# antoyang/FrozenBiLM

Hardware: AMD Instinct MI355X
Metric: video-text samples/sec (MLM fwd+bwd) DeBERTa-XL+adapters (higher is better)
Workload: dtype bf16; 1 GPU; DeBERTa-v2-XLarge(24L)+adapters ds8/8, B=32/GPU, T=10x1024, L=256 (S=266), MLM fwd+bwd+allreduce+clip+Adam, dropout 0.1 live, seeded random weights; global_batch=32, seq_len=266, parallelism=dp1, dead_layer23_encoder_pass=skipped (output unused, SURVEY fact 6); FLOPs still counted

## Files before the change

frozenbilm_amd/csrc/attn_bwd.hip:

```cpp
#include "attn_common.h"
#include "../../include/fbl.h"

namespace {
using namespace attn;

__global__ void rowdot_kernel(const bf16* dO, const bf16* O, long ld, float* out, int B, int S, int nh) {
  const long gid = (long)blockIdx.x * blockDim.x + threadIdx.x;
  const long idx = gid >> 3;
  const int c = (int)(gid & 7);
  const long total = (long)B * S * nh;
  const bool live = idx < total;
  const long row = live ? idx / nh : 0;
  const int h = live ? (int)(idx % nh) : 0;
  float s = 0.f;
  if (live) {
    const bf16x8 x = *(const bf16x8*)(dO + row * ld + h * 64 + c * 8);
    const bf16x8 y = *(const bf16x8*)(O + row * ld + h * 64 + c * 8);
#pragma unroll
    for (int e = 0; e < 8; ++e) s += bf2f(x[e]) * bf2f(y[e]);
  }
  s += __shfl_xor(s, 1, 64);
  s += __shfl_xor(s, 2, 64);
  s += __shfl_xor(s, 4, 64);
  if (live && c == 0) {
// ... 645 lines not shown
  }
}

struct BwdQArgs {
  const bf16* dS;
  const bf16* k; long ldk;
  const bf16* pkx;
  const int32_t* klen; const int32_t* border;
  bf16* dQ; long lddq;
  int B, S, Sp, nh;
  const int32_t* row0;
};
constexpr int LDG1 = 104;
constexpr int Q_DS = 0;
constexpr int Q_KS = Q_DS + 8192;
constexpr int Q_G1 = Q_KS + 8192;
constexpr int Q_TAB = Q_G1 + 64 * LDG1 * 2;
constexpr int Q_TOTAL = Q_TAB + 16384;
static_assert(3 * Q_TOTAL <= 160 * 1024, "three workgroups per CU");

template <bool PACKED = false>
__global__ __launch_bounds__(256, 3) void attn_bwd_dq_kernel(BwdQArgs a) {
  extern __shared__ __attribute__((aligned(16))) char smem[];
  const int tid = threadIdx.x, lane = tid & 63;
  const int w = __builtin_amdgcn_readfirstlane(tid >> 6);
  const int c = lane & 15, g = lane >> 4;
  const int S = a.S, Sp = a.Sp;
  const WgCoord wc = wg_coord(Sp / 64, a.nh, a.B, a.border);
  const int i0 = wc.x * 64, h = wc.h, b = wc.b;
  const int i = i0 + w * 16 + c;
  const long rb = PACKED ? (long)a.row0[b] : (long)b * S;
  const int lim = PACKED ? min(a.row0[b + 1] - a.row0[b], S) : S;
  const int kl = a.klen ? min(a.klen[b], S) : S;
  const int nkt = (i0 < kl) ? (kl + 63) / 64 : 0;
  const int srow = tid >> 3, sch = tid & 7;
  const int sb = srow * 128 + ((sch ^ tswz(srow)) << 4);
  const int ks0 = (w < 2) ? 0 : 1;
  bf16* g1 = (bf16*)(smem + Q_G1) + (w * 16 + c) * LDG1;
  const int wr = w * 16 + c;
  f32x4 dq[4];
#pragma unroll
  for (int dt = 0; dt < 4; ++dt) dq[dt] = (f32x4){0.f, 0.f, 0.f, 0.f};
  if (nkt > 0) {
    for (int t = tid; t < (64 * LDG1 * 2) / 16; t += 256) *(bf16x8*)(smem + Q_G1 + t * 16) = (bf16x8){0, 0, 0, 0, 0, 0, 0, 0};
    __syncthreads();
  }

  const long sbase = ((long)b * a.nh + h) * Sp * Sp;
  const __amdgpu_buffer_rsrc_t sr = buf_rsrc(a.dS + sbase + (long)i0 * Sp);
  const __amdgpu_buffer_rsrc_t kr = buf_rsrc(a.k + rb * a.ldk + h * 64);
  const __amdgpu_buffer_rsrc_t xr = buf_rsrc(a.pkx + (long)h * 2 * Sp * 64);
  const uint32_t so = (uint32_t)((wr * Sp + g * 16) * 2);
  const uint32_t ldk2 = (uint32_t)(a.ldk * 2);
  const int beta0 = (i0 - 64 + Sp) >> 6;

  struct Regs { bf16x8 s[2], k[2], x[2]; } R;
  auto load_pair = [&](int jt) {
#pragma unroll
    for (int t = 0; t < 2; ++t) {
      R.s[t] = buf_ld16(sr, so + (uint32_t)(t * 16), (uint32_t)(jt * 128));
      const uint32_t jr = (uint32_t)min(jt * 64 + srow + t * 32, lim - 1);
      R.k[t] = buf_ld16(kr, jr * ldk2 + (uint32_t)(sch * 16), 0);
      R.x[t] = buf_ld16(xr, (uint32_t)((srow + t * 32) * 128 + sch * 16), (uint32_t)((beta0 - jt) * 8192));
    }
  };
  if (nkt > 0) {
    load_pair(0);
#pragma unroll
    for (int t = 0; t < 2; ++t)
      *(bf16x8*)(smem + Q_TAB + ((beta0 + 1) & 1) * 8192 + sb + t * 4096) =
          buf_ld16(xr, (uint32_t)((srow + t * 32) * 128 + sch * 16), (uint32_t)((beta0 + 1) * 8192));
  }
  for (int jt = 0; jt < nkt; ++jt) {
#pragma unroll
    for (int t = 0; t < 2; ++t) {
      *(bf16x8*)(smem + Q_KS + sb + t * 4096) = R.k[t];
      *(bf16x8*)(smem + Q_TAB + ((beta0 - jt) & 1) * 8192 + sb + t * 4096) = R.x[t];
      *(bf16x8*)(smem + Q_DS + wr * 128 + (((2 * g + t) ^ (wr & 7)) << 4)) = R.s[t];
    }
    {
      bf16* gs = g1 + wr + 64 - g * 16 - ks0 * 32;
#pragma unroll
      for (int t = 0; t < 2; ++t)
#pragma unroll
        for (int e = 0; e < 8; ++e) gs[-(t * 8 + e)] = R.s[t][e];
    }
    __syncthreads();
    load_pair(min(jt + 1, nkt - 1));
#pragma unroll
    for (int kk = 0; kk < 2; ++kk) {
      const int rk = kk * 32 + g * 8 + (c >> 2);
      const bf16x8 sf = *(const bf16x8*)(smem + Q_DS + wr * 128 + (((kk * 4 + g) ^ (wr & 7)) << 4));
#pragma unroll
      for (int dt = 0; dt < 4; ++dt) {
        const int ch = dt * 2 + ((c >> 1) & 1), sub = (c & 1) * 8;
        union { tr16x4 h[2]; bf16x8 v; } u;
        u.h[0] = lds_tr16((const bf16*)(smem + Q_KS + rk * 128 + ((ch ^ tswz(rk)) << 4) + sub));
        u.h[1] = lds_tr16((const bf16*)(smem + Q_KS + (rk + 4) * 128 + ((ch ^ tswz(rk + 4)) << 4) + sub));
        dq[dt] = __builtin_amdgcn_mfma_f32_16x16x32_bf16(u.v, sf, dq[dt], 0, 0, 0);
      }
    }
#pragma unroll
    for (int u3 = 0; u3 < 3; ++u3) {
      const int x0 = (ks0 + u3) * 32 + g * 8;
      const int slot = ((beta0 - jt + (x0 >> 6)) & 1) * 8192;
      const int r = (x0 & 63) + (c >> 2);
      const bf16x8 gf = *(const bf16x8*)(g1 + u3 * 32 + g * 8);
#pragma unroll
      for (int dt = 0; dt < 4; ++dt) {
        const int ch = dt * 2 + ((c >> 1) & 1), sub = (c & 1) * 8;
        union { tr16x4 h[2]; bf16x8 v; } ut;
        ut.h[0] = lds_tr16((const bf16*)(smem + Q_TAB + slot + r * 128 + ((ch ^ tswz(r)) << 4) + sub));
        ut.h[1] = lds_tr16((const bf16*)(smem + Q_TAB + slot + (r + 4) * 128 + ((ch ^ tswz(r + 4)) << 4) + sub));
        dq[dt] = __builtin_amdgcn_mfma_f32_16x16x32_bf16(ut.v, gf, dq[dt], 0, 0, 0);
      }
    }
    __syncthreads();
  }
  if (i < lim) {
    bf16* op = a.dQ + (rb + i) * a.lddq + h * 64 + g * 4;
#pragma unroll
    for (int dt = 0; dt < 4; ++dt)
      *(bf16x4*)(op + dt * 16) = (bf16x4){f2bf(dq[dt][0]), f2bf(dq[dt][1]), f2bf(dq[dt][2]), f2bf(dq[dt][3])};
  }
}

struct ShearArgs {
  const bf16* X;
  const bf16* YT; long y_sh, y_sb, y_sd;
  const bf16* PT;
  const int16_t* relidx;
  const int32_t* klen;
  const int32_t* border;
  bf16* out; long ldout;
  int B, S, Sp, nh, span2, Wg;
  int lin;
  const int32_t* row0;
};
__device__ __forceinline__ void gt_window(const int16_t* relidx, int S, int kl, int r0, int Wg, int* rbase, int* nks) {
  const int hi = 2 * S - 2;
  const int dlo = -(r0 + 31), dhi = kl - 1 - r0;
  const int rb = (int)relidx[min(max(dlo + S - 1, 0), hi)] & ~7;
  const int rt = (int)relidx[min(max(dhi + S - 1, 0), hi)];
  *rbase = rb;
  *nks = min((rt - rb + 32) / 32, Wg / 32);
}
constexpr int C_IDX = 0;
constexpr int C_G = C_IDX + 2048;

template <bool PACKED = false>
__global__ __launch_bounds__(128) void attn_bwd_shear_kernel(ShearArgs a) {
  extern __shared__ __attribute__((aligned(16))) char smem[];
  const int tid = threadIdx.x, lane = tid & 63;
  const int w = __builtin_amdgcn_readfirstlane(tid >> 6);
  const int c = lane & 15, g = lane >> 4;
  const int S = a.S, Sp = a.Sp;
  const WgCoord wc = wg_coord(Sp / 32, a.nh, a.B, a.border);
  const int r0 = wc.x * 32, h = wc.h, b = wc.b;
  const int LDG = a.Wg + 8;
  const int rl = w * 16 + c;
  const int row = r0 + rl;
  bf16* G = (bf16*)(smem + C_G);
  int16_t* idx = (int16_t*)(smem + C_IDX);
  const bf16x8 z8 = {0, 0, 0, 0, 0, 0, 0, 0};
  const int kl = a.klen ? min(a.klen[b], S) : S;
  const long rb = PACKED ? (long)a.row0[b] : (long)b * S;
  const int lim = PACKED ? min(a.row0[b + 1] - a.row0[b], S) : S;
  if (r0 >= kl) {
    if (row < lim) {
      bf16* op = a.out + (rb + row) * a.ldout + h * 64 + g * 4;
#pragma unroll
      for (int dt = 0; dt < 4; ++dt) *(bf16x4*)(op + dt * 16) = (bf16x4){0, 0, 0, 0};
    }
    return;
  }
  int rbase, nks;
  gt_window(a.relidx, S, kl, r0, a.Wg, &rbase, &nks);
  const int izero = (int)a.relidx[S - 1];
  {
    const int vpr = nks * 4;
    for (int t = tid; t < 32 * vpr; t += 128) *(bf16x8*)(G + (t / vpr) * LDG + (t % vpr) * 8) = z8;
  }
  attn::load_idx_padded(idx, a.relidx, S, Sp, tid, 128);
  const long xbase = (((long)b * a.nh + h) * Sp + row) * Sp;
  f32x4 acc[4];
#pragma unroll
  for (int dt = 0; dt < 4; ++dt) acc[dt] = (f32x4){0.f, 0.f, 0.f, 0.f};
  __syncthreads();

  const int nct = (kl + 63) / 64;
  const bf16* ytb = a.YT + h * a.y_sh + b * a.y_sb + (long)c * a.y_sd + g * 8;
  const int16_t* ib = idx + (Sp - 1 - row + g * 8);
  bf16* grow = G + rl * LDG - rbase;
  const int wmax = rbase + nks * 32 - 1;
  const int dummy = rbase + a.Wg;
  const int lin0 = izero + g * 8 - row;
  const int rw = r0 + w * 16;
  struct Frags { bf16x8 y[8], x[2]; };
  auto load_ct = [&](int ct, Frags& F) {
    const int c0 = ct * 64;
#pragma unroll
    for (int kk = 0; kk < 2; ++kk)
#pragma unroll
      for (int dt = 0; dt < 4; ++dt)
        F.y[kk * 4 + dt] = (FBL_ATTN_DBGBITS & 2048) ? z8 : *(const bf16x8*)(ytb + (long)(dt * 16) * a.y_sd + c0 + kk * 32);
    F.x[0] = *(const bf16x8*)(a.X + xbase + c0 + g * 8);
    F.x[1] = *(const bf16x8*)(a.X + xbase + c0 + 32 + g * 8);
  };
  auto step = [&](int ct, const Frags& F) {
    const int c0 = ct * 64;
    const int d_a = rw - (c0 + 63), d_b = rw + 15 - c0;
    const bool band = max(abs(d_a), abs(d_b)) < a.lin;
#pragma unroll
    for (int kk = 0; kk < 2; ++kk) {
      const bf16x8 xv = F.x[kk];
#pragma unroll
      for (int dt = 0; dt < 4; ++dt) acc[dt] = __builtin_amdgcn_mfma_f32_16x16x32_bf16(F.y[kk * 4 + dt], xv, acc[dt], 0, 0, 0);
      const int cb = c0 + kk * 32;
      if (FBL_ATTN_DBGBITS & 512) continue;
      if (band) {
        const int s0 = lin0 + cb;
#pragma unroll
        for (int e = 0; e < 8; ++e) {
          const int slot = s0 + e;
          grow[bf2f(xv[e]) != 0.f ? slot : dummy] = xv[e];
        }
      } else {
#pragma unroll
        for (int e = 0; e < 8; ++e) {
          const float x = bf2f(xv[e]);
          if (x != 0.f) {
            const int dlt = cb + g * 8 + e - row;
            const int gi = clampi((int)ib[cb + e], rbase, wmax);
            if (abs(dlt) < a.lin) {
              grow[gi] = xv[e];
            } else {
              bf16x2 pv = {(bf16)0.f, (bf16)0.f};
              pv[gi & 1] = xv[e];
              __builtin_amdgcn_ds_atomic_fadd_v2bf16((__attribute__((address_space(3))) bf16x2*)(grow + (gi & ~1)), pv);
            }
          }
        }
      }
    }
  };
  {
    Frags F0, F1;
    load_ct(0, F0);
    for (int ct = 0; ct < nct; ct += 2) {
      if (ct + 1 < nct) load_ct(ct + 1, F1);
      step(ct, F0);
      if (ct + 2 < nct) load_ct(ct + 2, F0);
      if (ct + 1 < nct) step(ct + 1, F1);
    }
  }
  const bf16* pt = a.PT + (long)h * 64 * a.span2 + rbase + g * 8;
  auto load_pt = [&](int kk, bf16x8* dstf) {
#pragma unroll
    for (int dt = 0; dt < 4; ++dt) {
      const bool ok = rbase + kk * 32 + g * 8 + 8 <= a.span2;
      dstf[dt] = ok ? *(const bf16x8*)(pt + (long)(dt * 16 + c) * a.span2 + kk * 32) : z8;
    }
  };
  auto table_step = [&](int kk, const bf16x8* af) {
    const bf16x8 bfv = *(const bf16x8*)(G + rl * LDG + kk * 32 + g * 8);
#pragma unroll
    for (int dt = 0; dt < 4; ++dt) acc[dt] = __builtin_amdgcn_mfma_f32_16x16x32_bf16(af[dt], bfv, acc[dt], 0, 0, 0);
  };
  bf16x8 pa[4], pb[4];
  const int nks_run = (FBL_ATTN_DBGBITS & 1024) ? 0 : nks;
  load_pt(0, pa);
  for (int kk = 0; kk < nks_run; kk += 2) {
    if (kk + 1 < nks) load_pt(kk + 1, pb);
    table_step(kk, pa);
    if (kk + 2 < nks) load_pt(kk + 2, pa);
    if (kk + 1 < nks) table_step(kk + 1, pb);
  }
  if (row < lim) {
    bf16* op = a.out + (rb + row) * a.ldout + h * 64 + g * 4;
#pragma unroll
    for (int dt = 0; dt < 4; ++dt)
      *(bf16x4*)(op + dt * 16) = (bf16x4){f2bf(acc[dt][0]), f2bf(acc[dt][1]), f2bf(acc[dt][2]), f2bf(acc[dt][3])};
  }
}

constexpr int PG_MAX_E = 64;
struct PosGradArgs {
  const bf16* X[PG_MAX_E];
  const bf16* Y[PG_MAX_E];
  long ldy;
  const int16_t* dlo;
  const int16_t* dcnt;
  const int32_t* klen;
  const int32_t* row0;
  float* out;
  int E, B, S, Sp, nh, rcnt;
  int cmax;
};
constexpr int PG_PAD = 48;
constexpr int PG_LDY = 80;
constexpr int PG_TPW = 4;
constexpr int PG_WAVES = 4, PG_THR = PG_WAVES * 64;
constexpr int PG_ROWS = PG_WAVES * PG_TPW * 16;
__host__ __device__ constexpr int pg_pitch(int Sp) { return Sp + 2 * PG_PAD; }
__host__ __device__ constexpr int pg_buf(int Sp) { return 32 * pg_pitch(Sp) * 2 + 32 * PG_LDY * 2; }
__host__ __device__ constexpr int pg_smem(int Sp) { return 2 * pg_buf(Sp); }

template <bool NEG, int CM, int NXR, int OCC>
__global__ __launch_bounds__(PG_THR, OCC) void pos_grad_kernel(PosGradArgs a) {
  extern __shared__ __attribute__((aligned(16))) char smem[];
  const int tid = threadIdx.x, lane = tid & 63;
  const int w = __builtin_amdgcn_readfirstlane(tid >> 6);
  const int c = lane & 15, g = lane >> 4;
  const int S = a.S, Sp = a.Sp, P = pg_pitch(Sp);
  const int nsplit = (a.rcnt + PG_ROWS - 1) / PG_ROWS;
  const int L8 = blockIdx.x >> 3, xcd = blockIdx.x & 7;
  const int prob = (L8 / nsplit) * 8 + xcd, part = L8 % nsplit;
  if (prob >= a.E * a.nh) return;
  const int e = prob / a.nh, h = prob % a.nh;
  const int bufsz = pg_buf(Sp);
  const bf16* X = a.X[e];
  const bf16* Y = a.Y[e];
  const int ntiles = (a.rcnt + 15) / 16;

  int d0[PG_TPW], dn[PG_TPW], tlo[PG_TPW], thi[PG_TPW];
  bool simple[PG_TPW];
#pragma unroll
  for (int u = 0; u < PG_TPW; ++u) {
    const int t = (w + PG_WAVES * u) * nsplit + part;
    const int r = min(t * 16 + c, a.rcnt - 1);
    const bool live = t < ntiles && t * 16 + c < a.rcnt;
    d0[u] = live ? (int)a.dlo[r] : 0;
    dn[u] = live ? (int)a.dcnt[r] : 0;
    const int rf = min(t * 16, a.rcnt - 1), rl = min(t * 16 + 15, a.rcnt - 1);
    tlo[u] = t < ntiles ? (int)a.dlo[rf] : 1 << 20;
    thi[u] = t < ntiles ? (int)a.dlo[rl] + (int)a.dcnt[rl] - 1 : -(1 << 20);
    simple[u] = t < ntiles && t * 16 + 15 < a.rcnt && (thi[u] - tlo[u]) == 15 && __builtin_amdgcn_ballot_w64(dn[u] != 1) == 0;
  }
  f32x4 acc[PG_TPW][4];
#pragma unroll
  for (int u = 0; u < PG_TPW; ++u)
#pragma unroll
    for (int dt = 0; dt < 4; ++dt) acc[u][dt] = (f32x4){0.f, 0.f, 0.f, 0.f};

  for (int id = tid; id < (OCC >= 3 ? 1 : 2) * 32 * 2 * (PG_PAD / 8); id += PG_THR) {
    const int bsel = id / (32 * 2 * (PG_PAD / 8)), r2 = id % (32 * 2 * (PG_PAD / 8));
    const int row = r2 / (2 * (PG_PAD / 8)), q = r2 % (2 * (PG_PAD / 8));
    const int col = q < PG_PAD / 8 ? q * 8 : PG_PAD + Sp + (q - PG_PAD / 8) * 8;
    *(bf16x8*)((bf16*)(smem + bsel * bufsz) + row * P + col) = (bf16x8){0, 0, 0, 0, 0, 0, 0, 0};
  }
  const bf16x8 z8 = (bf16x8){0, 0, 0, 0, 0, 0, 0, 0};
  const int srow = tid >> 3, sch = tid & 7, nq = Sp >> 6;

  int b_n = 0, k_n = 0, kl_n = 0;
  auto seek = [&]() {
    while (b_n < a.B) {
      kl_n = a.klen ? min(a.klen[b_n], S) : S;
      if (k_n < kl_n) return true;
      ++b_n; k_n = 0;
    }
    return false;
  };
  bf16x8 rx[NXR], ry;
  int it_b = 0, it_k = 0, it_kl = 0;
  auto load_item = [&]() {
    it_b = b_n; it_k = k_n; it_kl = kl_n;
    const int kl64 = (kl_n + 63) & ~63;
    const long rb = a.row0 ? (long)a.row0[b_n] : (long)b_n * S;
    const int lim = a.row0 ? min(a.row0[b_n + 1] - a.row0[b_n], S) : S;
    const bf16* Xb = X + (((long)b_n * a.nh + h) * Sp) * Sp + (long)k_n * Sp;
    const bf16* xr = Xb + (long)srow * Sp + sch * 8;
#pragma unroll
    for (int q = 0; q < NXR; ++q) rx[q] = (q < nq && sch * 8 + q * 64 < kl64) ? *(const bf16x8*)(xr + q * 64) : z8;
    {
      const int pos = k_n + srow;
      ry = (pos < lim) ? *(const bf16x8*)(Y + (rb + pos) * a.ldy + h * 64 + sch * 8) : z8;
    }
    k_n += 32;
  };
  int pb = 0;
  bool have = seek();
  if (have) load_item();
  while (have) {
    bf16* xs = (bf16*)(smem + pb * bufsz);
    bf16* ys = xs + 32 * P;
    if (OCC >= 3) __syncthreads();
    {
      bf16* xw = xs + srow * P + PG_PAD + sch * 8;
#pragma unroll
      for (int q = 0; q < NXR; ++q)
        if (q < nq) *(bf16x8*)(xw + q * 64) = rx[q];
    }
    *(bf16x8*)(ys + srow * PG_LDY + sch * 8) = ry;
    const int k0 = it_k, kl = it_kl;
    __syncthreads();
    have = seek();
    if (have) load_item();
    bf16x8 yf[4];
#pragma unroll
    for (int dt = 0; dt < 4; ++dt) {
      const bf16* yb = ys + (g * 8 + (c >> 2)) * PG_LDY + dt * 16 + (c & 3) * 4;
      union { tr16x4 hh[2]; bf16x8 v; } u2;
      u2.hh[0] = lds_tr16(yb);
      u2.hh[1] = lds_tr16(yb + 4 * PG_LDY);
      yf[dt] = u2.v;
    }
#pragma unroll
    for (int u = 0; u < PG_TPW; ++u) {
      const int cmin = NEG ? k0 + tlo[u] : k0 - thi[u];
      const int cmax = NEG ? k0 + 31 + thi[u] : k0 + 31 - tlo[u];
      if (cmax < 0 || cmin >= kl) continue;
      bf16x8 gf;
      const bf16* xrow = xs + (g * 8) * P + PG_PAD;
      const int cb = NEG ? (k0 + g * 8 + d0[u]) : (k0 + g * 8 - d0[u]);
      if (simple[u]) {
#pragma unroll
        for (int q = 0; q < 8; ++q) gf[q] = xrow[q * P + cb + q];
      } else {
        const int lo = -PG_PAD, hi = Sp + PG_PAD - 1;
        bf16 vv[8][CM];
#pragma unroll
        for (int q = 0; q < 8; ++q)
#pragma unroll
          for (int t2 = 0; t2 < CM; ++t2) vv[q][t2] = xrow[q * P + clampi(NEG ? cb + q + t2 : cb + q - t2, lo, hi)];
#pragma unroll
        for (int q = 0; q < 8; ++q) {
          float sum = 0.f;
#pragma unroll
          for (int t2 = 0; t2 < CM; ++t2) sum += t2 < dn[u] ? bf2f(vv[q][t2]) : 0.f;
          gf[q] = f2bf(sum);
        }
      }
#pragma unroll
      for (int dt = 0; dt < 4; ++dt) acc[u][dt] = __builtin_amdgcn_mfma_f32_16x16x32_bf16(yf[dt], gf, acc[u][dt], 0, 0, 0);
    }
    if (OCC < 3) pb ^= 1;
  }
  float* ob = a.out + ((long)e * a.nh + h) * a.rcnt * 64;
#pragma unroll
  for (int u = 0; u < PG_TPW; ++u) {
    const int r = ((w + PG_WAVES * u) * nsplit + part) * 16 + c;
    if (r < a.rcnt) {
#pragma unroll
      for (int dt = 0; dt < 4; ++dt) *(f32x4*)(ob + (long)r * 64 + dt * 16 + g * 4) = acc[u][dt];
    }
  }
}

constexpr int PGW_PAD = 6;
__host__ __device__ constexpr int pgw_pitch(int Sp) { return Sp + PGW_PAD; }
__host__ __device__ constexpr int pgw_smem(int Sp) { return 32 * pgw_pitch(Sp) * 4 + 32 * PG_LDY * 2; }

template <bool NEG>
__global__ __launch_bounds__(PG_THR, 2) void pos_grad_wide_kernel(PosGradArgs a) {
  extern __shared__ __attribute__((aligned(16))) char smem[];
  const int tid = threadIdx.x, lane = tid & 63;
  const int w = __builtin_amdgcn_readfirstlane(tid >> 6);
  const int c = lane & 15, g = lane >> 4;
  const int S = a.S, Sp = a.Sp, PP = pgw_pitch(Sp);
  const int nsplit = (a.rcnt + PG_ROWS - 1) / PG_ROWS;
  const int L8 = blockIdx.x >> 3, xcd = blockIdx.x & 7;
  const int prob = (L8 / nsplit) * 8 + xcd, part = L8 % nsplit;
  if (prob >= a.E * a.nh) return;
  const int e = prob / a.nh, h = prob % a.nh;
  float* cs = (float*)smem;
  bf16* ys = (bf16*)(smem + 32 * PP * 4);
  const bf16* X = a.X[e];
  const bf16* Y = a.Y[e];
  const int ntiles = (a.rcnt + 15) / 16;

  int d0[PG_TPW], dn[PG_TPW], tlo[PG_TPW], thi[PG_TPW];
#pragma unroll
  for (int u = 0; u < PG_TPW; ++u) {
    const int t = (w + PG_WAVES * u) * nsplit + part;
    const int r = min(t * 16 + c, a.rcnt - 1);
    const bool live = t < ntiles && t * 16 + c < a.rcnt;
    d0[u] = live ? (int)a.dlo[r] : 0;
    dn[u] = live ? (int)a.dcnt[r] : 0;
    const int rf = min(t * 16, a.rcnt - 1), rl = min(t * 16 + 15, a.rcnt - 1);
    tlo[u] = t < ntiles ? (int)a.dlo[rf] : 1 << 20;
    thi[u] = t < ntiles ? (int)a.dlo[rl] + (int)a.dcnt[rl] - 1 : -(1 << 20);
  }
  f32x4 acc[PG_TPW][4];
#pragma unroll
  for (int u = 0; u < PG_TPW; ++u)
#pragma unroll
    for (int dt = 0; dt < 4; ++dt) acc[u][dt] = (f32x4){0.f, 0.f, 0.f, 0.f};

  if (tid < 32) cs[tid * PP + 1] = 0.f;
  const bf16x8 z8 = (bf16x8){0, 0, 0, 0, 0, 0, 0, 0};
  const int srow = tid >> 3, sch = tid & 7, nq = Sp >> 6;

  int b_n = 0, k_n = 0, kl_n = 0;
  auto seek = [&]() {
    while (b_n < a.B) {
      kl_n = a.klen ? min(a.klen[b_n], S) : S;
      if (k_n < kl_n) return true;
      ++b_n; k_n = 0;
    }
    return false;
  };
  bf16x8 rx[8], ry;
  int it_k = 0, it_kl = 0;
  auto load_item = [&]() {
    it_k = k_n; it_kl = kl_n;
    const int kl64 = (kl_n + 63) & ~63;
    const long rb = a.row0 ? (long)a.row0[b_n] : (long)b_n * S;
    const int lim = a.row0 ? min(a.row0[b_n + 1] - a.row0[b_n], S) : S;
    const bf16* xr = X + (((long)b_n * a.nh + h) * Sp) * Sp + (long)(k_n + srow) * Sp + sch * 8;
#pragma unroll
    for (int q = 0; q < 8; ++q) rx[q] = (q < nq && sch * 8 + q * 64 < kl64) ? *(const bf16x8*)(xr + q * 64) : z8;
    const int pos = k_n + srow;
    ry = (pos < lim) ? *(const bf16x8*)(Y + (rb + pos) * a.ldy + h * 64 + sch * 8) : z8;
    k_n += 32;
  };
  bool have = seek();
  if (have) load_item();
  while (have) {
    __syncthreads();
    {
      float* cw = cs + srow * PP + 2 + sch * 8;
      float carry = 0.f;
#pragma unroll
      for (int q = 0; q < 8; ++q) {
        if (q < nq) {
          float run[8];
          run[0] = bf2f(rx[q][0]);
#pragma unroll
          for (int i = 1; i < 8; ++i) run[i] = run[i - 1] + bf2f(rx[q][i]);
          float incl = run[7];
#pragma unroll
          for (int s = 1; s < 8; s <<= 1) {
            const float o = __shfl_up(incl, s, 8);
            if (sch >= s) incl += o;
          }
          const float excl = __shfl_up(incl, 1, 8);
          const float base = carry + (sch ? excl : 0.f);
#pragma unroll
          for (int i = 0; i < 8; i += 2) *(float2*)(cw + q * 64 + i) = make_float2(base + run[i], base + run[i + 1]);
          carry += __shfl(incl, 7, 8);
        }
      }
    }
    *(bf16x8*)(ys + srow * PG_LDY + sch * 8) = ry;
    const int k0 = it_k, kl = it_kl;
    __syncthreads();
    have = seek();
    if (have) load_item();
    bf16x8 yf[4];
#pragma unroll
    for (int dt = 0; dt < 4; ++dt) {
      const bf16* yb = ys + (g * 8 + (c >> 2)) * PG_LDY + dt * 16 + (c & 3) * 4;
      union { tr16x4 hh[2]; bf16x8 v; } u2;
      u2.hh[0] = lds_tr16(yb);
      u2.hh[1] = lds_tr16(yb + 4 * PG_LDY);
      yf[dt] = u2.v;
    }
    const float* crow = cs + (g * 8) * PP + 1;
#pragma unroll
    for (int u = 0; u < PG_TPW; ++u) {
      const int cmin = NEG ? k0 + tlo[u] : k0 - thi[u];
      const int cmax = NEG ? k0 + 31 + thi[u] : k0 + 31 - tlo[u];
      if (cmax < 0 || cmin >= kl) continue;
      const int kb = k0 + g * 8;
      float hi[8], lo[8];
#pragma unroll
      for (int q = 0; q < 8; ++q) {
        const int jl = NEG ? kb + q + d0[u] : kb + q - d0[u] - dn[u] + 1;
        hi[q] = crow[q * PP + clampi(jl + dn[u], 0, Sp)];
        lo[q] = crow[q * PP + clampi(jl, 0, Sp)];
      }
      bf16x8 gf;
#pragma unroll
      for (int q = 0; q < 8; ++q) gf[q] = f2bf(hi[q] - lo[q]);
#pragma unroll
      for (int dt = 0; dt < 4; ++dt) acc[u][dt] = __builtin_amdgcn_mfma_f32_16x16x32_bf16(yf[dt], gf, acc[u][dt], 0, 0, 0);
    }
  }
  float* ob = a.out + ((long)e * a.nh + h) * a.rcnt * 64;
#pragma unroll
  for (int u = 0; u < PG_TPW; ++u) {
    const int r = ((w + PG_WAVES * u) * nsplit + part) * 16 + c;
    if (r < a.rcnt) {
#pragma unroll
      for (int dt = 0; dt < 4; ++dt) *(f32x4*)(ob + (long)r * 64 + dt * 16 + g * 4) = acc[u][dt];
    }
  }
}

}

extern "C" int fbl_attn_rowdot(const void* dO, const void* O, int64_t ld, float* out, int B, int S, int nh,
                               void* stream) {
  if (ld % 8) return FBL_ERR_ALIGN;
  const long total = (long)B * S * nh;
  if (total <= 0) return 0;
  hipLaunchKernelGGL(rowdot_kernel, dim3((unsigned)((total * 8 + 255) / 256)), dim3(256), 0, (hipStream_t)stream,
                     (const bf16*)dO, (const bf16*)O, (long)ld, out, B, S, nh);
  FBL_CHECK_LAUNCH();
  return 0;
}

extern "C" int fbl_disent_attn_bwd_ds(const void* q, const void* k, const void* v, int64_t ldq, const void* dO,
                                      int64_t ldo,
                                      const void* pk, const void* pq, int64_t ldp, const int16_t* relidx,
                                      const int32_t* mask, const int32_t* klen, const int32_t* border, const float* lse, const float* Dv, float scale, float p_drop,
                                      uint64_t seed, const uint64_t* seed_dev, void* dV, int64_t lddv, void* dS, void* dST, int B, int S, int Sp,
                                      int nh, int span2, int lin_span, const int32_t* row0, void* stream) {
  if (!grid_shape_ok(S, Sp)) return FBL_ERR_SHAPE;
  if ((ldq % 8) || (ldo % 8) || (ldp % 8) || (lddv % 4)) return FBL_ERR_ALIGN;
  if (lin_span < 0 || 2 * lin_span > span2) return FBL_ERR_ARG;
  if (row0 && !klen) return FBL_ERR_ARG;
  if (B <= 0 || nh <= 0) return 0;
  BwdAArgs a{};
  a.q = (const bf16*)q; a.k = (const bf16*)k; a.v = (const bf16*)v; a.ldq = ldq;
  a.dO = (const bf16*)dO; a.ldo = ldo;
  a.pk = (const bf16*)pk; a.pq = (const bf16*)pq; a.ldp = ldp;
  a.relidx = relidx; a.mask = mask; a.klen = klen; a.border = border;
  a.lse = lse; a.Dv = Dv;
  a.scale = scale; a.p_drop = p_drop; a.seed = seed; a.seed_dev = seed_dev;
  a.dV = (bf16*)dV; a.lddv = lddv; a.dS = (bf16*)dS; a.dST = (bf16*)dST;
  a.B = B; a.S = S; a.Sp = Sp; a.nh = nh; a.span2 = span2; a.lin = lin_span;
  a.row0 = row0;
  attn_debug_init();
  const dim3 grid((unsigned)(Sp / 64) * nh * B);
  return fbl_bool(seed_dev && p_drop > 0.f, [&](auto DEVSEED) {
    return fbl_bool(row0 != nullptr, [&](auto PACKED) {
      return fbl_launch<attn_bwd_ds_kernel<decltype(DEVSEED)::value, decltype(PACKED)::value>>(grid, dim3(256), a_total(Sp),
                                                                                               stream, a);
    });
  });
}

extern "C" int fbl_disent_attn_bwd_dspk(const void* psave, const float* msave, const void* q, int64_t ldq, const void* v, int64_t ldv,
                                        const void* dO, int64_t ldo, const void* pqx, const int32_t* klen, const int32_t* border,
                                        const float* lse, const float* Dv, float scale, float p_drop, uint64_t seed,
                                        const uint64_t* seed_dev, void* dK, int64_t lddk, void* dV, int64_t lddv, void* dS, void* dST,
                                        int B, int S, int Sp, int nh, const int32_t* row0, void* stream) {
  if (!grid_shape_ok(S, Sp)) return FBL_ERR_SHAPE;
  if ((ldv % 8) || (ldo % 8) || (ldq % 8) || (lddv % 4) || (lddk % 4)) return FBL_ERR_ALIGN;
  if (!psave || !msave || !q || !v || !dO || !pqx || !lse || !Dv || !dK || !dV || !dS || !dST) return FBL_ERR_ARG;
  if (row0 && !klen) return FBL_ERR_ARG;
  if (B <= 0 || nh <= 0) return 0;
  BwdPKArgs a{};
  a.p.psave = (const bf16*)psave; a.p.msave = msave;
  a.p.v = (const bf16*)v; a.p.ldv = ldv; a.p.dO = (const bf16*)dO; a.p.ldo = ldo;
  a.p.klen = klen; a.p.border = border; a.p.lse = lse; a.p.Dv = Dv;
  a.p.scale = scale; a.p.p_drop = p_drop; a.p.seed = seed; a.p.seed_dev = seed_dev;
  a.p.dV = (bf16*)dV; a.p.lddv = lddv; a.p.dS = (bf16*)dS; a.p.dST = (bf16*)dST;
  a.p.B = B; a.p.S = S; a.p.Sp = Sp; a.p.nh = nh; a.p.row0 = row0;
  a.q = (const bf16*)q; a.ldq = ldq; a.pqx = (const bf16*)pqx; a.dK = (bf16*)dK; a.lddk = lddk;
  attn_debug_init();
  const dim3 grid((unsigned)(Sp / 64) * nh * B);
  return fbl_bool(row0 != nullptr, [&](auto PACKED) {
    return fbl_launch<attn_bwd_dspk_kernel<decltype(PACKED)::value>>(grid, dim3(256), K_TOTAL, stream, a);
  });
}

extern "C" int fbl_disent_attn_bwd_dq(const void* dS, const void* k, int64_t ldk, const void* pkx, const int32_t* klen,
                                      const int32_t* border, void* dQ, int64_t lddq, int B, int S, int Sp, int nh,
                                      const int32_t* row0, void* stream) {
  if (!grid_shape_ok(S, Sp)) return FBL_ERR_SHAPE;
  if ((ldk % 8) || (lddq % 4)) return FBL_ERR_ALIGN;
  if (!dS || !k || !pkx || !dQ) return FBL_ERR_ARG;
  if (row0 && !klen) return FBL_ERR_ARG;
  if (B <= 0 || nh <= 0) return 0;
  BwdQArgs a{(const bf16*)dS, (const bf16*)k, ldk, (const bf16*)pkx, klen, border, (bf16*)dQ, lddq, B, S, Sp, nh, row0};
  const dim3 grid((unsigned)(Sp / 64) * nh * B);
  return fbl_bool(row0 != nullptr, [&](auto PACKED) {
    return fbl_launch<attn_bwd_dq_kernel<decltype(PACKED)::value>>(grid, dim3(256), Q_TOTAL, stream, a);
  });
}

extern "C" int fbl_disent_attn_bwd_shear(const void* dST, const void* QT, int64_t y_sh, int64_t y_sb, int64_t y_sd,
                                         const void* PQT, const int16_t* relidx, const int32_t* klen, const int32_t* border,
                                         void* dK, int64_t lddk, int lin_span, int B, int S, int Sp, int nh, int span2,
                                         const int32_t* row0, void* stream) {
  if (!grid_shape_ok(S, Sp) || span2 > 512 || span2 % 32) return FBL_ERR_SHAPE;
  if ((lddk % 4) || (y_sd % 8) || (y_sb % 8) || (y_sh % 8)) return FBL_ERR_ALIGN;
  if (B <= 0 || nh <= 0) return 0;
  if (row0 && !klen) return FBL_ERR_ARG;
  ShearArgs a{};
  a.X = (const bf16*)dST;
  a.YT = (const bf16*)QT; a.y_sh = y_sh; a.y_sb = y_sb; a.y_sd = y_sd;
  a.PT = (const bf16*)PQT;
  a.relidx = relidx; a.klen = klen; a.border = border;
  a.out = (bf16*)dK; a.ldout = lddk;
  a.B = B; a.S = S; a.Sp = Sp; a.nh = nh; a.span2 = span2; a.lin = lin_span;
  a.row0 = row0;
  a.Wg = S + 31 + 7;
  if (a.Wg > span2) a.Wg = span2;
  a.Wg = (a.Wg + 31) / 32 * 32;
  attn_debug_init();
  const dim3 grid((unsigned)(Sp / 32) * nh * B);
  return fbl_bool(row0 != nullptr, [&](auto PACKED) {
    return fbl_launch<attn_bwd_shear_kernel<decltype(PACKED)::value>>(grid, dim3(128), C_G + 32 * (a.Wg + 8) * 2, stream, a);
  });
}

extern "C" int fbl_attn_pos_grad(int neg, const void* const* X, const void* const* Y, int64_t ldy, const int16_t* dlo,
                                 const int16_t* dcnt, int dcnt_max, const int32_t* klen, const int32_t* row0, float* out, int E,
                                 int B, int S, int Sp, int nh, int rcnt, void* stream) {
  if (!grid_shape_ok(S, Sp) || rcnt < 1 || rcnt > 1024) return FBL_ERR_SHAPE;
  if (ldy % 8) return FBL_ERR_ALIGN;
  if (!X || !Y || !dlo || !dcnt || !out || dcnt_max < 1) return FBL_ERR_ARG;
  if (row0 && !klen) return FBL_ERR_ARG;
  if (E <= 0 || B <= 0 || nh <= 0) return 0;
  for (int e = 0; e < E; ++e)
    if (!X[e] || !Y[e]) return FBL_ERR_ARG;
  static const int occ_sw = FBL_ENV_INT("FBL_POSGRAD_OCC", 3);
  const bool occ3 = Sp <= 320 && dcnt_max <= 3 && occ_sw >= 3;
  const bool wide = dcnt_max > 8;
  const int nsplit = (rcnt + PG_ROWS - 1) / PG_ROWS;
  for (int e0 = 0; e0 < E; e0 += PG_MAX_E) {
    PosGradArgs a{};
    const int ne = E - e0 < PG_MAX_E ? E - e0 : PG_MAX_E;
    for (int e = 0; e < ne; ++e) {
      a.X[e] = (const bf16*)X[e0 + e];
      a.Y[e] = (const bf16*)Y[e0 + e];
    }
    a.ldy = ldy; a.dlo = dlo; a.dcnt = dcnt; a.klen = klen; a.row0 = row0;
    a.out = out + (long)e0 * nh * rcnt * 64;
    a.E = ne; a.B = B; a.S = S; a.Sp = Sp; a.nh = nh; a.rcnt = rcnt; a.cmax = dcnt_max;
    const dim3 grid((unsigned)(((ne * nh + 7) / 8) * 8 * nsplit)), block(PG_THR);
    const int rc = fbl_bool(neg != 0, [&](auto NEG) {
      constexpr bool N = decltype(NEG)::value;
      if (wide) return fbl_launch<pos_grad_wide_kernel<N>>(grid, block, pgw_smem(Sp), stream, a);
      if (occ3) return fbl_launch<pos_grad_kernel<N, 3, 5, 3>>(grid, block, pg_buf(Sp), stream, a);
      if (dcnt_max <= 3) return fbl_launch<pos_grad_kernel<N, 3, 8, 2>>(grid, block, pg_smem(Sp), stream, a);
      return fbl_launch<pos_grad_kernel<N, 8, 8, 2>>(grid, block, pg_smem(Sp), stream, a);
    });
    if (rc) return rc;
  }
  return 0;
}

extern "C" int fbl_attn_bwd_prep(const void* q, int64_t ldq, const void* pq, const void* pk, int64_t ldp, const void* dO,
                                 const void* O, int64_t ldo, void* QT, void* PQT, float* Dv, const int16_t* relidx, void* PQX,
                                 void* PKX, int B, int S, int Sp, int nh, int span2, const int32_t* row0, void* stream) {
  if (S < 1 || Sp < S || Sp % 64 || span2 <= 0 || span2 % 64) return FBL_ERR_SHAPE;
  if ((ldq % 8) || (ldp % 8) || (ldo % 8)) return FBL_ERR_ALIGN;
  if ((PQX || PKX) && !relidx) return FBL_ERR_ARG;
  if (!Dv) return FBL_ERR_ARG;
  if (B <= 0 || nh <= 0) return 0;
  const int n_tr = (Sp / 64) * nh * B, n_tab = (span2 / 64) * nh, n_x = (2 * Sp / 64) * nh;
  PrepArgs a{};
  a.q = (const bf16*)q; a.ldq = ldq;
  a.pq = (const bf16*)pq; a.pk = (const bf16*)pk; a.ldp = ldp;
  a.dO = (const bf16*)dO; a.O = (const bf16*)O; a.ldo = ldo;
  a.QT = (bf16*)QT; a.PQT = (bf16*)PQT; a.Dv = Dv;
  a.B = B; a.S = S; a.Sp = Sp; a.nh = nh; a.span2 = span2;
  a.n_qt = QT ? n_tr : 0; a.n_pqt = PQT ? n_tab : 0;
  a.row0 = row0; a.relidx = relidx;
  a.PQX = (bf16*)PQX; a.PKX = (bf16*)PKX;
  a.n_pqx = PQX ? n_x : 0; a.n_pkx = PKX ? n_x : 0;
  const long n_dot = ((long)B * S * nh * 8 + 255) / 256;
  const long grid = (long)a.n_qt + a.n_pqt + a.n_pqx + a.n_pkx + n_dot;
  hipLaunchKernelGGL(attn_bwd_prep_kernel, dim3((unsigned)grid), dim3(256), 0, (hipStream_t)stream, a);
  FBL_CHECK_LAUNCH();
  return 0;
}
```

Measured before the change: 811.6 samples/s.

## Cut register pressure and LDS bank conflicts in positional-gradient kernel

Result: faster. 825.2 samples/s, median of 6 (+1.7%).

```diff
diff --git a/frozenbilm_amd/csrc/attn_bwd.hip b/frozenbilm_amd/csrc/attn_bwd.hip
--- a/frozenbilm_amd/csrc/attn_bwd.hip
+++ b/frozenbilm_amd/csrc/attn_bwd.hip
@@ -971,11 +971,19 @@
 constexpr int PG_TPW = 4;
 constexpr int PG_WAVES = 4, PG_THR = PG_WAVES * 64;
 constexpr int PG_ROWS = PG_WAVES * PG_TPW * 16;
+constexpr int PG_TPR = PG_THR / 32;
+constexpr int PG_YV = 64 / PG_TPR;
+typedef bf16 pg_yvec __attribute__((ext_vector_type(PG_YV)));
+typedef __attribute__((address_space(4))) const int32_t pg_cint;
+constexpr int PG_NXR_SHORT = 384 / (8 * PG_TPR), PG_NXR_LONG = 512 / (8 * PG_TPR);
+constexpr int PG_GOFF = 24;
 __host__ __device__ constexpr int pg_pitch(int Sp) { return Sp + 2 * PG_PAD; }
-__host__ __device__ constexpr int pg_buf(int Sp) { return 32 * pg_pitch(Sp) * 2 + 32 * PG_LDY * 2; }
-__host__ __device__ constexpr int pg_smem(int Sp) { return 2 * pg_buf(Sp); }
-
-template <bool NEG, int CM, int NXR, int OCC>
+constexpr int PG_DD = PG_ROWS * 4;
+__host__ __device__ constexpr int pg_buf(int Sp) {
+  return (32 * pg_pitch(Sp) + 4 * PG_GOFF) * 2 + 32 * PG_LDY * 2;
+}
+
+template <bool NEG, int CM, int NXR, int OCC, bool DB>
 __global__ __launch_bounds__(PG_THR, OCC) void pos_grad_kernel(PosGradArgs a) {
   extern __shared__ __attribute__((aligned(16))) char smem[];
   const int tid = threadIdx.x, lane = tid & 63;
@@ -986,25 +994,26 @@
   const int L8 = blockIdx.x >> 3, xcd = blockIdx.x & 7;
   const int prob = (L8 / nsplit) * 8 + xcd, part = L8 % nsplit;
   if (prob >= a.E * a.nh) return;
-  const int e = prob / a.nh, h = prob % a.nh;
+  const int e = __builtin_amdgcn_readfirstlane(prob / a.nh), h = __builtin_amdgcn_readfirstlane(prob % a.nh);
   const int bufsz = pg_buf(Sp);
   const bf16* X = a.X[e];
   const bf16* Y = a.Y[e];
   const int ntiles = (a.rcnt + 15) / 16;
 
-  int d0[PG_TPW], dn[PG_TPW], tlo[PG_TPW], thi[PG_TPW];
+  int* ddp = (int*)(smem + (DB ? 2 : 1) * bufsz) + w * 16 + c;
+  int tlo[PG_TPW], thi[PG_TPW];
   bool simple[PG_TPW];
 #pragma unroll
   for (int u = 0; u < PG_TPW; ++u) {
     const int t = (w + PG_WAVES * u) * nsplit + part;
     const int r = min(t * 16 + c, a.rcnt - 1);
     const bool live = t < ntiles && t * 16 + c < a.rcnt;
-    d0[u] = live ? (int)a.dlo[r] : 0;
-    dn[u] = live ? (int)a.dcnt[r] : 0;
+    const int d0 = live ? (int)a.dlo[r] : 0, dn = live ? (int)a.dcnt[r] : 0;
+    ddp[u * PG_WAVES * 16] = (d0 & 0xffff) | (dn << 16);
     const int rf = min(t * 16, a.rcnt - 1), rl = min(t * 16 + 15, a.rcnt - 1);
-    tlo[u] = t < ntiles ? (int)a.dlo[rf] : 1 << 20;
-    thi[u] = t < ntiles ? (int)a.dlo[rl] + (int)a.dcnt[rl] - 1 : -(1 << 20);
-    simple[u] = t < ntiles && t * 16 + 15 < a.rcnt && (thi[u] - tlo[u]) == 15 && __builtin_amdgcn_ballot_w64(dn[u] != 1) == 0;
+    tlo[u] = __builtin_amdgcn_readfirstlane(t < ntiles ? (int)a.dlo[rf] : 1 << 20);
+    thi[u] = __builtin_amdgcn_readfirstlane(t < ntiles ? (int)a.dlo[rl] + (int)a.dcnt[rl] - 1 : -(1 << 20));
+    simple[u] = t < ntiles && t * 16 + 15 < a.rcnt && (thi[u] - tlo[u]) == 15 && __builtin_amdgcn_ballot_w64(dn != 1) == 0;
   }
   f32x4 acc[PG_TPW][4];
 #pragma unroll
@@ -1012,59 +1021,72 @@
 #pragma unroll
     for (int dt = 0; dt < 4; ++dt) acc[u][dt] = (f32x4){0.f, 0.f, 0.f, 0.f};
 
-  for (int id = tid; id < (OCC >= 3 ? 1 : 2) * 32 * 2 * (PG_PAD / 8); id += PG_THR) {
+  for (int id = tid; id < (DB ? 2 : 1) * 32 * 2 * (PG_PAD / 8); id += PG_THR) {
     const int bsel = id / (32 * 2 * (PG_PAD / 8)), r2 = id % (32 * 2 * (PG_PAD / 8));
     const int row = r2 / (2 * (PG_PAD / 8)), q = r2 % (2 * (PG_PAD / 8));
     const int col = q < PG_PAD / 8 ? q * 8 : PG_PAD + Sp + (q - PG_PAD / 8) * 8;
-    *(bf16x8*)((bf16*)(smem + bsel * bufsz) + row * P + col) = (bf16x8){0, 0, 0, 0, 0, 0, 0, 0};
+    *(bf16x8*)((bf16*)(smem + bsel * bufsz) + row * P + (row >> 3) * PG_GOFF + col) = (bf16x8){0, 0, 0, 0, 0, 0, 0, 0};
   }
   const bf16x8 z8 = (bf16x8){0, 0, 0, 0, 0, 0, 0, 0};
-  const int srow = tid >> 3, sch = tid & 7, nq = Sp >> 6;
-
-  int b_n = 0, k_n = 0, kl_n = 0;
+  const int srow = tid / PG_TPR, sch = tid % PG_TPR;
+
+  const int B = a.B;
+  const pg_cint* klc = (const pg_cint*)a.klen;
+  const pg_cint* r0c = (const pg_cint*)a.row0;
+  auto klen_raw = [&](int b) { return b < B ? (klc ? klc[b] : S) : 0; };
+  int b_n = 0, k_n = 0, kl_n = min(klen_raw(0), S), kl_x = klen_raw(1);
   auto seek = [&]() {
-    while (b_n < a.B) {
-      kl_n = a.klen ? min(a.klen[b_n], S) : S;
-      if (k_n < kl_n) return true;
+    while (b_n < B && k_n >= kl_n) {
       ++b_n; k_n = 0;
-    }
-    return false;
+      kl_n = min(kl_x, S);
+      kl_x = klen_raw(b_n + 1);
+    }
+    return b_n < B;
   };
-  bf16x8 rx[NXR], ry;
-  int it_b = 0, it_k = 0, it_kl = 0;
+  bf16x8 rx[NXR];
+  pg_yvec ry;
+  int it_k = 0, it_kl = 0;
   auto load_item = [&]() {
-    it_b = b_n; it_k = k_n; it_kl = kl_n;
+    it_k = k_n; it_kl = kl_n;
     const int kl64 = (kl_n + 63) & ~63;
-    const long rb = a.row0 ? (long)a.row0[b_n] : (long)b_n * S;
-    const int lim = a.row0 ? min(a.row0[b_n + 1] - a.row0[b_n], S) : S;
-    const bf16* Xb = X + (((long)b_n * a.nh + h) * Sp) * Sp + (long)k_n * Sp;
-    const bf16* xr = Xb + (long)srow * Sp + sch * 8;
-#pragma unroll
-    for (int q = 0; q < NXR; ++q) rx[q] = (q < nq && sch * 8 + q * 64 < kl64) ? *(const bf16x8*)(xr + q * 64) : z8;
+    const int bb = min(b_n, B - 1);
+    const bf16* xr = X + (((long)bb * a.nh + h) * Sp + k_n + srow) * Sp;
+#pragma unroll
+    for (int q = 0; q < NXR; ++q) {
+      const int col = (sch + PG_TPR * q) * 8;
+      const bool ok = col < kl64;
+      const bf16x8 v = *(const bf16x8*)(xr + (ok ? col : (sch & 7) * 8));
+      rx[q] = ok ? v : z8;
+    }
     {
+      const long rb = r0c ? (long)r0c[bb] : (long)bb * S;
+      const int lim = r0c ? min(r0c[bb + 1] - r0c[bb], S) : S;
       const int pos = k_n + srow;
-      ry = (pos < lim) ? *(const bf16x8*)(Y + (rb + pos) * a.ldy + h * 64 + sch * 8) : z8;
+      const bf16* yb = Y + rb * a.ldy + h * 64;
+      ry = (pos < lim) ? *(const pg_yvec*)(yb + (unsigned)pos * (unsigned)a.ldy + sch * PG_YV) : pg_yvec{};
     }
     k_n += 32;
   };
   int pb = 0;
   bool have = seek();
-  if (have) load_item();
+  load_item();
   while (have) {
     bf16* xs = (bf16*)(smem + pb * bufsz);
-    bf16* ys = xs + 32 * P;
-    if (OCC >= 3) __syncthreads();
+    bf16* ys = xs + 32 * P + 4 * PG_GOFF;
+    if (!DB) __syncthreads();
     {
-      bf16* xw = xs + srow * P + PG_PAD + sch * 8;
-#pragma unroll
-      for (int q = 0; q < NXR; ++q)
-        if (q < nq) *(bf16x8*)(xw + q * 64) = rx[q];
-    }
-    *(bf16x8*)(ys + srow * PG_LDY + sch * 8) = ry;
+      bf16* xw = xs + srow * P + (srow >> 3) * PG_GOFF + PG_PAD;
+#pragma unroll
+      for (int q = 0; q < NXR; ++q) {
+        const int col = (sch + PG_TPR * q) * 8;
+        if (col < Sp) *(bf16x8*)(xw + col) = rx[q];
+      }
+    }
+    *(pg_yvec*)(ys + srow * PG_LDY + sch * PG_YV) = ry;
     const int k0 = it_k, kl = it_kl;
     __syncthreads();
     have = seek();
-    if (have) load_item();
+    load_item();
     bf16x8 yf[4];
 #pragma unroll
     for (int dt = 0; dt < 4; ++dt) {
@@ -1080,30 +1102,36 @@
       const int cmax = NEG ? k0 + 31 + thi[u] : k0 + 31 - tlo[u];
       if (cmax < 0 || cmin >= kl) continue;
       bf16x8 gf;
-      const bf16* xrow = xs + (g * 8) * P + PG_PAD;
-      const int cb = NEG ? (k0 + g * 8 + d0[u]) : (k0 + g * 8 - d0[u]);
+      const bf16* xrow = xs + (g * 8) * P + g * PG_GOFF + PG_PAD;
+      const int dd = ddp[u * PG_WAVES * 16];
+      const int d0 = (int)(int16_t)dd, dn = dd >> 16;
+      const int cb = NEG ? (k0 + g * 8 + d0) : (k0 + g * 8 - d0);
       if (simple[u]) {
 #pragma unroll
         for (int q = 0; q < 8; ++q) gf[q] = xrow[q * P + cb + q];
       } else {
         const int lo = -PG_PAD, hi = Sp + PG_PAD - 1;
-        bf16 vv[8][CM];
-#pragma unroll
-        for (int q = 0; q < 8; ++q)
-#pragma unroll
-          for (int t2 = 0; t2 < CM; ++t2) vv[q][t2] = xrow[q * P + clampi(NEG ? cb + q + t2 : cb + q - t2, lo, hi)];
-#pragma unroll
-        for (int q = 0; q < 8; ++q) {
-          float sum = 0.f;
-#pragma unroll
-          for (int t2 = 0; t2 < CM; ++t2) sum += t2 < dn[u] ? bf2f(vv[q][t2]) : 0.f;
-          gf[q] = f2bf(sum);
+#pragma unroll
+        for (int qh = 0; qh < 8; qh += 4) {
+          bf16 vv[4][CM];
+#pragma unroll
+          for (int q = 0; q < 4; ++q)
+#pragma unroll
+            for (int t2 = 0; t2 < CM; ++t2)
+              vv[q][t2] = xrow[(qh + q) * P + clampi(NEG ? cb + qh + q + t2 : cb + qh + q - t2, lo, hi)];
+#pragma unroll
+          for (int q = 0; q < 4; ++q) {
+            float sum = 0.f;
+#pragma unroll
+            for (int t2 = 0; t2 < CM; ++t2) sum += t2 < dn ? bf2f(vv[q][t2]) : 0.f;
+            gf[qh + q] = f2bf(sum);
+          }
         }
       }
 #pragma unroll
       for (int dt = 0; dt < 4; ++dt) acc[u][dt] = __builtin_amdgcn_mfma_f32_16x16x32_bf16(yf[dt], gf, acc[u][dt], 0, 0, 0);
     }
-    if (OCC < 3) pb ^= 1;
+    if (DB) pb ^= 1;
   }
   float* ob = a.out + ((long)e * a.nh + h) * a.rcnt * 64;
 #pragma unroll
@@ -1117,17 +1145,18 @@
 }
 
 constexpr int PGW_PAD = 6;
+constexpr int PGW_TPW = 4, PGW_WAVES = 4, PGW_THR = PGW_WAVES * 64, PGW_ROWS = PGW_WAVES * PGW_TPW * 16;
 __host__ __device__ constexpr int pgw_pitch(int Sp) { return Sp + PGW_PAD; }
 __host__ __device__ constexpr int pgw_smem(int Sp) { return 32 * pgw_pitch(Sp) * 4 + 32 * PG_LDY * 2; }
 
 template <bool NEG>
-__global__ __launch_bounds__(PG_THR, 2) void pos_grad_wide_kernel(PosGradArgs a) {
+__global__ __launch_bounds__(PGW_THR, 2) void pos_grad_wide_kernel(PosGradArgs a) {
   extern __shared__ __attribute__((aligned(16))) char smem[];
   const int tid = threadIdx.x, lane = tid & 63;
   const int w = __builtin_amdgcn_readfirstlane(tid >> 6);
   const int c = lane & 15, g = lane >> 4;
   const int S = a.S, Sp = a.Sp, PP = pgw_pitch(Sp);
-  const int nsplit = (a.rcnt + PG_ROWS - 1) / PG_ROWS;
+  const int nsplit = (a.rcnt + PGW_ROWS - 1) / PGW_ROWS;
   const int L8 = blockIdx.x >> 3, xcd = blockIdx.x & 7;
   const int prob = (L8 / nsplit) * 8 + xcd, part = L8 % nsplit;
   if (prob >= a.E * a.nh) return;
@@ -1138,10 +1167,10 @@
   const bf16* Y = a.Y[e];
   const int ntiles = (a.rcnt + 15) / 16;
 
-  int d0[PG_TPW], dn[PG_TPW], tlo[PG_TPW], thi[PG_TPW];
-#pragma unroll
-  for (int u = 0; u < PG_TPW; ++u) {
-    const int t = (w + PG_WAVES * u) * nsplit + part;
+  int d0[PGW_TPW], dn[PGW_TPW], tlo[PGW_TPW], thi[PGW_TPW];
+#pragma unroll
+  for (int u = 0; u < PGW_TPW; ++u) {
+    const int t = (w + PGW_WAVES * u) * nsplit + part;
     const int r = min(t * 16 + c, a.rcnt - 1);
     const bool live = t < ntiles && t * 16 + c < a.rcnt;
     d0[u] = live ? (int)a.dlo[r] : 0;
@@ -1150,9 +1179,9 @@
     tlo[u] = t < ntiles ? (int)a.dlo[rf] : 1 << 20;
     thi[u] = t < ntiles ? (int)a.dlo[rl] + (int)a.dcnt[rl] - 1 : -(1 << 20);
   }
-  f32x4 acc[PG_TPW][4];
-#pragma unroll
-  for (int u = 0; u < PG_TPW; ++u)
+  f32x4 acc[PGW_TPW][4];
+#pragma unroll
+  for (int u = 0; u < PGW_TPW; ++u)
 #pragma unroll
     for (int dt = 0; dt < 4; ++dt) acc[u][dt] = (f32x4){0.f, 0.f, 0.f, 0.f};
 
@@ -1227,7 +1256,7 @@
     }
     const float* crow = cs + (g * 8) * PP + 1;
 #pragma unroll
-    for (int u = 0; u < PG_TPW; ++u) {
+    for (int u = 0; u < PGW_TPW; ++u) {
       const int cmin = NEG ? k0 + tlo[u] : k0 - thi[u];
       const int cmax = NEG ? k0 + 31 + thi[u] : k0 + 31 - tlo[u];
       if (cmax < 0 || cmin >= kl) continue;
@@ -1248,8 +1277,8 @@
   }
   float* ob = a.out + ((long)e * a.nh + h) * a.rcnt * 64;
 #pragma unroll
-  for (int u = 0; u < PG_TPW; ++u) {
-    const int r = ((w + PG_WAVES * u) * nsplit + part) * 16 + c;
+  for (int u = 0; u < PGW_TPW; ++u) {
+    const int r = ((w + PGW_WAVES * u) * nsplit + part) * 16 + c;
     if (r < a.rcnt) {
 #pragma unroll
       for (int dt = 0; dt < 4; ++dt) *(f32x4*)(ob + (long)r * 64 + dt * 16 + g * 4) = acc[u][dt];
@@ -1372,15 +1401,18 @@
                                  int B, int S, int Sp, int nh, int rcnt, void* stream) {
   if (!grid_shape_ok(S, Sp) || rcnt < 1 || rcnt > 1024) return FBL_ERR_SHAPE;
   if (ldy % 8) return FBL_ERR_ALIGN;
+  if (ldy < 64 || ldy >= (1 << 21)) return FBL_ERR_SHAPE;
   if (!X || !Y || !dlo || !dcnt || !out || dcnt_max < 1) return FBL_ERR_ARG;
   if (row0 && !klen) return FBL_ERR_ARG;
   if (E <= 0 || B <= 0 || nh <= 0) return 0;
   for (int e = 0; e < E; ++e)
     if (!X[e] || !Y[e]) return FBL_ERR_ARG;
-  static const int occ_sw = FBL_ENV_INT("FBL_POSGRAD_OCC", 3);
-  const bool occ3 = Sp <= 320 && dcnt_max <= 3 && occ_sw >= 3;
   const bool wide = dcnt_max > 8;
-  const int nsplit = (rcnt + PG_ROWS - 1) / PG_ROWS;
+  const int nsplit = (rcnt + (wide ? PGW_ROWS : PG_ROWS) - 1) / (wide ? PGW_ROWS : PG_ROWS);
+  const bool occ3 = Sp <= 320 && dcnt_max <= 3;
+  const bool db = Sp <= 384;
+  static_assert(2 * (2 * pg_buf(384) + PG_DD) <= 160 * 1024, "two double-buffered workgroups per CU");
+  static_assert(PG_TPR * 8 * PG_NXR_LONG >= 512 && PG_TPR * 8 * PG_NXR_SHORT >= 384, "chunks per thread cover the row");
   for (int e0 = 0; e0 < E; e0 += PG_MAX_E) {
     PosGradArgs a{};
     const int ne = E - e0 < PG_MAX_E ? E - e0 : PG_MAX_E;
@@ -1391,13 +1423,16 @@
     a.ldy = ldy; a.dlo = dlo; a.dcnt = dcnt; a.klen = klen; a.row0 = row0;
     a.out = out + (long)e0 * nh * rcnt * 64;
     a.E = ne; a.B = B; a.S = S; a.Sp = Sp; a.nh = nh; a.rcnt = rcnt; a.cmax = dcnt_max;
-    const dim3 grid((unsigned)(((ne * nh + 7) / 8) * 8 * nsplit)), block(PG_THR);
+    const dim3 grid((unsigned)(((ne * nh + 7) / 8) * 8 * nsplit)), block(wide ? PGW_THR : PG_THR);
     const int rc = fbl_bool(neg != 0, [&](auto NEG) {
       constexpr bool N = decltype(NEG)::value;
       if (wide) return fbl_launch<pos_grad_wide_kernel<N>>(grid, block, pgw_smem(Sp), stream, a);
-      if (occ3) return fbl_launch<pos_grad_kernel<N, 3, 5, 3>>(grid, block, pg_buf(Sp), stream, a);
-      if (dcnt_max <= 3) return fbl_launch<pos_grad_kernel<N, 3, 8, 2>>(grid, block, pg_smem(Sp), stream, a);
-      return fbl_launch<pos_grad_kernel<N, 8, 8, 2>>(grid, block, pg_smem(Sp), stream, a);
+      if (occ3) return fbl_launch<pos_grad_kernel<N, 3, 5, 3, false>>(grid, block, pg_buf(Sp) + PG_DD, stream, a);
+      if (dcnt_max <= 3)
+        return db ? fbl_launch<pos_grad_kernel<N, 3, PG_NXR_SHORT, 2, true>>(grid, block, 2 * pg_buf(Sp) + PG_DD, stream, a)
+                  : fbl_launch<pos_grad_kernel<N, 3, PG_NXR_LONG, 2, false>>(grid, block, pg_buf(Sp) + PG_DD, stream, a);
+      return db ? fbl_launch<pos_grad_kernel<N, 8, PG_NXR_SHORT, 2, true>>(grid, block, 2 * pg_buf(Sp) + PG_DD, stream, a)
+                : fbl_launch<pos_grad_kernel<N, 8, PG_NXR_LONG, 2, false>>(grid, block, pg_buf(Sp) + PG_DD, stream, a);
     });
     if (rc) return rc;
   }
```
